# henreedev/audio-pathtracer

Hardware: AMD Instinct MI355X
Metric: rays/sec + IR-frames/sec (1s IR, depth 8) (higher is better)
Workload: dtype f32

## Files before the change

### audio-pathtracer_amd/csrc/fs_aux_kernels.hip

```cpp
#include "fs_dev_trav.hpp"
#include "fs_dev_walk.hpp"
#include "fs_dev_coop.hpp"
#include "fs_dev_recon.hpp"
#include "fs_launch.hpp"

namespace fs {
namespace {

template <bool SPECTRAL>
__global__ __launch_bounds__(kBlock) void reconstruct_kernel(const float* __restrict__ energy, int B, int nb,
                                                             int num_samples, int spb, float* __restrict__ ir_bands,
                                                             float* __restrict__ ir_mono, const float* __restrict__ carrier) {
    extern __shared__ __attribute__((aligned(16))) float s_amp[];
    if (SPECTRAL && (int)blockIdx.y == B) {
        reconstruct_spectral_row((int)blockIdx.x, energy, B, nb, num_samples, spb, ir_bands, ir_mono, s_amp, nullptr, nullptr, carrier);
        return;
    }
    reconstruct_body_fast((int)blockIdx.y, (int)blockIdx.x, energy, B, nb, num_samples, spb, ir_bands, ir_mono, s_amp, nullptr);
}

template <bool SPECTRAL>
__global__ __launch_bounds__(kBlock) void reconstruct_batch_kernel(const ReconItem* __restrict__ table, int B, int nb, int num_samples,
                                                                   uint32_t cb, PublishWord pub, const float* __restrict__ carrier) {
    extern __shared__ __attribute__((aligned(16))) float s_rb[];
// ... 244 lines not shown
                    finished = false;
                }
            }
            if (finished) {
                if (is_occl) { acc->occlusion = de; mode = DONE; }
                else { if (de > 0.0f) { ++direct_hits; direct_sum += de; } mode = MAIN; }
            }
        }
    }
    if (mine && !is_occl) {
        if (result > 0.0f) atomicAdd(&acc->reaching, 1u);
        if (direct_hits) { atomicAdd(&acc->direct_hits, direct_hits); atomicAdd(&acc->direct_energy_sum, direct_sum); }
    }
    if (traces) atomicAdd(&acc->traces, traces);
}

__global__ void add_energy_kernel(float* row, int nb, float delay, float e) {
    float x = (delay * 1000.f) / 1.0f;
    float fl = floorf(x);
    int bin = !(fl > 0.0f) ? 0 : (fl >= (float)(nb - 1) ? nb - 1 : (int)fl);
    row[bin] += e;
}

}

void launch_reconstruct(const float* energy, int B, int num_bins, int sample_rate, int num_samples, int spb,
                        float* ir_bands, float* ir_mono, hipStream_t s, const float* carrier) {
    (void)sample_rate;
    int chunks = (num_samples + kChunk - 1) / kChunk;
    dim3 grid((chunks + kBlock - 1) / kBlock, B + 1);
    const size_t lds = recon_lds_bytes(num_bins);
    if (carrier) {
        allow_lds(reconstruct_kernel<true>, lds);
        hipLaunchKernelGGL(reconstruct_kernel<true>, grid, dim3(kBlock), lds, s, energy, B, num_bins, num_samples, spb, ir_bands, ir_mono, carrier);
    } else {
        allow_lds(reconstruct_kernel<false>, lds);
        hipLaunchKernelGGL(reconstruct_kernel<false>, grid, dim3(kBlock), lds, s, energy, B, num_bins, num_samples, spb, ir_bands, ir_mono, nullptr);
    }
}

void launch_reconstruct_batch(const ReconItem* table, int count, int B, int num_bins, int num_samples, hipStream_t s, const PublishWord& pub,
                              const float* carrier, float* const* room, float bin_duration) {
    if (count <= 0) return;
    const uint32_t chunks = (uint32_t)((num_samples + kChunk - 1) / kChunk), cb = (chunks + kBlock - 1) / kBlock;
    const size_t lds = recon_lds_bytes(num_bins);
    bool spectral = false;
// ... 101 lines not shown
```

### audio-pathtracer_amd/csrc/fs_capi_context.cpp

```cpp
#include "fs_context.hpp"

#include <chrono>

namespace fsi {

Source* get_source(fs_context* ctx, fs_source h) {
    if (h < 0 || (size_t)h >= ctx->sources.size()) return nullptr;
    Source* s = ctx->sources[(size_t)h];
    return (s && s->alive) ? s : nullptr;
}

hipError_t compute_waits_for(fs_context* ctx, hipEvent_t ev) {
    const hipError_t q = hipEventQuery(ev);
    if (q == hipSuccess) { ctx->dbg.waits_skipped++; return hipSuccess; }
    (void)hipGetLastError();
    ctx->dbg.waits_enqueued++;
    return hipStreamWaitEvent(ctx->stream, ev, 0);
}
hipEvent_t tail_batch_event(fs_context* ctx, uint64_t id) {
    const uint64_t newest = ctx->tail_batch_newest.load(std::memory_order_acquire);
    const uint64_t probe = newest - id < (uint64_t)fs_context::kTailBatches ? id : newest - fs_context::kTailBatches + 1;
    return ctx->tail_batch_ev[probe % fs_context::kTailBatches];
}
bool tail_batch_done(fs_context* ctx, uint64_t id) {
// ... 132 lines not shown
    ctx->coop16_nodes = 0; ctx->coop_levels = 0;
    if (ctx->d_tris) (void)hipFree(ctx->d_tris);
    if (ctx->d_tris48) (void)hipFree(ctx->d_tris48);
    if (ctx->d_tri_nrm) (void)hipFree(ctx->d_tri_nrm);
    if (ctx->d_absorption) (void)hipFree(ctx->d_absorption);
    if (ctx->d_leaf_pos) (void)hipFree(ctx->d_leaf_pos);
    if (ctx->d_node_box) (void)hipFree(ctx->d_node_box);
    if (ctx->d_move) (void)hipFree(ctx->d_move);
    ctx->d_leaf_pos = nullptr; ctx->d_node_box = nullptr; ctx->d_move = nullptr;
    ctx->move_cap = 0;
    ctx->refit_pending = false;
    ctx->d_nodes = nullptr; ctx->d_tris = nullptr; ctx->d_absorption = nullptr;
    ctx->d_tris48 = nullptr; ctx->d_tri_nrm = nullptr;
    if (ctx->deep.buf) (void)hipFree(ctx->deep.buf);
    for (int32_t* b : ctx->deep.retired) (void)hipFree(b);
    ctx->deep = DeepStore{};
    ctx->scene = DeviceScene{};
    ctx->committed = false;
}

void free_state(fs_context* ctx) {
    if (ctx->st.end_pos) (void)hipFree(ctx->st.end_pos);
    if (ctx->st.end_misc) (void)hipFree(ctx->st.end_misc);
    if (ctx->st.seg_np) (void)hipFree(ctx->st.seg_np);
    if (ctx->st.seg_mat) (void)hipFree(ctx->st.seg_mat);
    if (ctx->d_seg_pos) (void)hipFree(ctx->d_seg_pos);
    ctx->d_seg_pos = nullptr; ctx->cap_pos = 0;
    if (ctx->st.slot_of) (void)hipFree(ctx->st.slot_of);
    for (void* q : {(void*)ctx->d_over_np, (void*)ctx->d_over_mat, (void*)ctx->d_over_pos, (void*)ctx->d_cont, (void*)ctx->d_end_posd})
        if (q) (void)hipFree(q);
    if (ctx->h_overflow) (void)hipHostFree(ctx->h_overflow);
    ctx->h_overflow = nullptr;
    ctx->d_over_np = nullptr; ctx->d_over_mat = nullptr; ctx->d_over_pos = nullptr; ctx->d_overflow = nullptr; ctx->d_cont = nullptr; ctx->d_end_posd = nullptr;
    ctx->over_cap = ctx->over_cap_pos = 0; ctx->cap_posd = 0;
    if (ctx->walk.perm) (void)hipFree(ctx->walk.perm);
    ctx->walk.perm = nullptr;
    ctx->st = SubpathState{};
    ctx->cap_lanes = ctx->cap_seg = 0;
}

hipEvent_t take_event(fs_context* ctx) {
    if (!ctx->free_events.empty()) {
        hipEvent_t e = ctx->free_events.back();
        ctx->free_events.pop_back();
        return e;
    }
// ... 67 lines not shown
        want_cap = (uint32_t)std::min<size_t>(lanes, std::max<size_t>(ctx->over_cap, (size_t)(4.0 * tail * (double)lanes) + 64));
        if (ctx->over_cap_forced > 0) want_cap = std::max(ctx->over_cap, (uint32_t)ctx->over_cap_forced);
    }
    const bool new_sets = sets != ctx->state_sets || staged != ctx->state_cont;
    const bool grow_lanes = lanes > ctx->cap_lanes || new_sets;
    const bool grow_seg = seg > ctx->cap_seg || grow_lanes;
    const bool grow_over = unbounded && (want_cap > ctx->over_cap || !ctx->d_over_np || new_sets);
    const bool grow_over_pos = unbounded && want_positions && (want_cap > ctx->over_cap_pos || !ctx->d_over_pos);
    const bool grow_pos = want > ctx->cap_pos;
    if (grow_lanes || grow_seg || grow_over || grow_over_pos || grow_pos) {
        FS_FLUSH(ctx);
        FS_HIP(ctx, hipStreamSynchronize(ctx->stream));
    }
    if (grow_pos) {
        if (ctx->d_seg_pos) (void)hipFree(ctx->d_seg_pos);
        ctx->d_seg_pos = nullptr; ctx->cap_pos = 0;
        FS_HIP(ctx, hipMalloc((void**)&ctx->d_seg_pos, sizeof(float4) * std::max<size_t>(want, 1)));
        ctx->cap_pos = want;
    }
    if (grow_lanes) {
        lanes = std::max(lanes, ctx->cap_lanes);
        if (ctx->st.end_pos) (void)hipFree(ctx->st.end_pos);
        if (ctx->st.end_misc) (void)hipFree(ctx->st.end_misc);
        if (ctx->st.slot_of) (void)hipFree(ctx->st.slot_of);
        if (ctx->walk.perm) (void)hipFree(ctx->walk.perm);
        if (ctx->d_cont) (void)hipFree(ctx->d_cont);
        ctx->st.end_pos = nullptr; ctx->st.end_misc = nullptr; ctx->st.slot_of = nullptr; ctx->d_cont = nullptr;
        ctx->walk.perm = nullptr;
        ctx->cap_lanes = 0;
        FS_HIP(ctx, hipMalloc((void**)&ctx->st.end_pos, sizeof(float4) * (size_t)sets * lanes));
        FS_HIP(ctx, hipMalloc((void**)&ctx->st.end_misc, sizeof(uint2) * (size_t)sets * lanes));
        FS_HIP(ctx, hipMalloc((void**)&ctx->st.slot_of, sizeof(uint32_t) * (size_t)sets * lanes));
        if (staged) FS_HIP(ctx, hipMalloc((void**)&ctx->d_cont, sizeof(float4) * 2 * (size_t)sets * lanes));
        ctx->cap_seg = 0;
        ctx->cap_lanes = lanes;
        ctx->state_sets = sets;
        ctx->state_cont = staged;
    }
    if (grow_seg) {
        seg = std::max(seg, (size_t)levels * ctx->cap_lanes);
        if (ctx->st.seg_np) (void)hipFree(ctx->st.seg_np);
        if (ctx->st.seg_mat) (void)hipFree(ctx->st.seg_mat);
        ctx->st.seg_np = nullptr; ctx->st.seg_mat = nullptr;
        ctx->cap_seg = 0;
        FS_HIP(ctx, hipMalloc((void**)&ctx->st.seg_np, sizeof(float2) * (size_t)ctx->state_sets * seg));
        FS_HIP(ctx, hipMalloc((void**)&ctx->st.seg_mat, sizeof(uint32_t) * (size_t)ctx->state_sets * seg));
        if (ctx->walk.perm) (void)hipFree(ctx->walk.perm);
        ctx->walk.perm = nullptr;
        ctx->perm_words = seg + ctx->cap_lanes;
        FS_HIP(ctx, hipMalloc((void**)&ctx->walk.perm, sizeof(uint32_t) * (size_t)ctx->state_sets * ctx->perm_words));
        ctx->cap_seg = seg;
    }
    if (!ctx->d_overflow) {
        FS_HIP(ctx, hipHostMalloc((void**)&ctx->h_overflow, 64, hipHostMallocDefault));
// ... 389 lines not shown
```

### audio-pathtracer_amd/csrc/fs_capi_frame.cpp

```cpp
#include "fs_context.hpp"

namespace {

int ensure_energy_buffer(fs_context* ctx, Source* s, int b) {
    if (s->d_energy[b]) return FS_OK;
    const size_t eb = sizeof(float) * (size_t)ctx->cfg.num_bands * (size_t)ctx->num_bins;
    FS_HIP(ctx, hipMalloc((void**)&s->d_energy[b], eb));
    FS_HIP(ctx, hipMemsetAsync(s->d_energy[b], 0, eb, ctx->stream));
    if (!s->ev_rec[b]) FS_HIP(ctx, hipEventCreateWithFlags(&s->ev_rec[b], kDeviceEventFlags));
    if (!s->ev_red[b]) FS_HIP(ctx, hipEventCreateWithFlags(&s->ev_red[b], kDeviceEventFlags));
    return FS_OK;
}

struct Frame {
    Source* const* srcs = nullptr;
    int count = 0;
    const fs_params* p = nullptr;
    const fs_context::GroupEntry* group = nullptr;
    KParams kp{};
    int B = 1, levels = 0;
    bool batch = false, unbounded = false, all_conn = false, mis = false, fixed = false, accumulate = false, pipe_ok = false;
    bool dir = false;
    DirArgs dargs{};
    std::vector<WalkStage> stages;
// ... 109 lines not shown
        std::vector<int> own_bound;
        const bool lane = (ctx->coop_info.wide16.rec != nullptr || ctx->coop_info.wide4.rec != nullptr) && sync_lane_plan(ctx, kp, &f.lane_len, &lane_bound);
        if (!lane) f.lane_len = 0;
        if (lane && ctx->sync_stage_bounds_default && lane_bound > 0) own_bound.push_back(lane_bound);
        for (int bound : own_bound.empty() ? ctx->sync_stage_bounds : own_bound) { WalkStage sr; sr.begin = begin; sr.end = bound; f.stages.push_back(sr); begin = bound; }
        WalkStage last; last.begin = begin; last.end = 1 << 30;
        f.stages.push_back(last);
    } else {
        f.stages.push_back(WalkStage());
    }
}

int frame_resources(fs_context* ctx, Frame& f) {
    KParams& kp = f.kp;
    const int B = f.B, count = f.count;
    const bool staged = f.stages.size() > 1;
    int rc = ensure_state(ctx, kp.num_local, f.levels, f.unbounded, (double)f.p->rr_prob, f.all_conn, f.mis,
                          (int)f.stages.size() + 2, staged);
    if (rc) return rc;
    f.fidx = ctx->frame_index;
    const size_t set = f.fidx % (unsigned)ctx->state_sets;
    SubpathState& st = f.st;
    st = ctx->st;
    st.end_pos += set * ctx->cap_lanes; st.end_misc += set * ctx->cap_lanes; st.slot_of += set * ctx->cap_lanes;
    st.seg_np += set * ctx->cap_seg; st.seg_mat += set * ctx->cap_seg;
    st.cont_a = staged ? ctx->d_cont + 2 * set * ctx->cap_lanes : nullptr;
    st.cont_b = staged ? st.cont_a + ctx->cap_lanes : nullptr;
    st.end_posd = nullptr;
    if (kp.dpos) {
        const size_t lanes = 2 * (size_t)kp.num_local;
        if (lanes > ctx->cap_posd) {
            FS_HIP(ctx, hipStreamSynchronize(ctx->stream));
            if (ctx->d_end_posd) (void)hipFree(ctx->d_end_posd);
            ctx->d_end_posd = nullptr; ctx->cap_posd = 0;
            FS_HIP(ctx, hipMalloc((void**)&ctx->d_end_posd, sizeof(double) * 3 * lanes));
            ctx->cap_posd = lanes;
        }
        st.end_posd = ctx->d_end_posd;
    }
    f.scratch = ctx->walk.queue_head + (size_t)(f.fidx % kScratchSets) * kScratchAllocWords;
    f.perm_buf = ctx->walk.perm ? ctx->walk.perm + set * ctx->perm_words : nullptr;
    st.seg_pos = f.all_conn ? ctx->d_seg_pos : nullptr;
    st.seg_nrm = f.mis ? ctx->d_seg_pos + (size_t)f.levels * 2 * (size_t)kp.num_local : nullptr;
    st.main_levels = f.levels;
    st.over_levels = f.unbounded ? kOverLevels : 0;
    st.over_cap = f.unbounded ? ctx->over_cap : 0;
    st.over_np = ctx->d_over_np ? ctx->d_over_np + set * (size_t)kOverLevels * ctx->over_cap : nullptr;
// ... 657 lines not shown
```

### audio-pathtracer_amd/csrc/fs_capi_scene.cpp

```cpp
#include "fs_context.hpp"

static int update_triangles(fs_context* ctx, int32_t first, int32_t count, const float* xyz, bool new_rest);

namespace fsi {

void cancel_refine(fs_context* ctx) {
    if (ctx->refine) ctx->refine->cancel.store(true, std::memory_order_relaxed);
    ctx->refine.reset();
    ctx->moved_since_refine = false;
}
void wait_refine(const std::shared_ptr<RefineJob>& j) {
    std::unique_lock<std::mutex> l(j->mu);
    j->cv.wait(l, [&] { return j->done; });
}
void join_refine_threads(fs_context* ctx) {
    for (std::thread& t : ctx->refine_threads)
        if (t.joinable()) t.join();
    ctx->refine_threads.clear();
}

static inline void transform_vertex(const float* a, const float* r, float* w) {
    const float x = r[0], y = r[1], z = r[2];
    for (int k = 0; k < 3; ++k) w[k] = ((a[4 * k] * x + a[4 * k + 1] * y) + a[4 * k + 2] * z) + a[4 * k + 3];
}
// ... 94 lines not shown
}

int fs_scene_set_materials(fs_context* ctx, const float* absorption, const float* transmission,
                           const float* scattering, int32_t M, int32_t B) {
    if (!ctx) return FS_ERR_INVALID_ARGUMENT;
    if (M < 0 || (M > 0 && !absorption) || M >= (int32_t)FS_NO_MATERIAL)
        return ctx->fail(FS_ERR_INVALID_ARGUMENT, "bad material table");
    if (B != ctx->cfg.num_bands) return ctx->fail(FS_ERR_SIZE_MISMATCH, "material bands != context num_bands");
    size_t n = (size_t)M * (size_t)B;
    ctx->h_absorption.assign(absorption, absorption + n);
    if (transmission) ctx->h_transmission.assign(transmission, transmission + n); else ctx->h_transmission.clear();
    if (scattering) ctx->h_scattering.assign(scattering, scattering + n); else ctx->h_scattering.clear();
    ctx->M = M;
    ctx->committed = false;
    return FS_OK;
}

static int upload_materials(fs_context* ctx) {
    const size_t mb = ctx->h_absorption.size() * sizeof(float);
    if (mb) {
        const int B = ctx->cfg.num_bands, M = ctx->M;
        std::vector<float> table(ctx->h_absorption);
        table.resize((size_t)M * B + (size_t)M * 3 * B + (size_t)M * 3, 0.f);
        float* gain = table.data() + (size_t)M * B;
        float* prob = gain + (size_t)M * 3 * B;
        const bool has_t = ctx->h_transmission.size() == (size_t)M * B, has_s = ctx->h_scattering.size() == (size_t)M * B;
        for (int m = 0; m < M; ++m) {
            float sum[3] = {0.f, 0.f, 0.f};
            for (int b = 0; b < B; ++b) {
                const float alpha = ctx->h_absorption[(size_t)m * B + b];
                float tau = has_t ? ctx->h_transmission[(size_t)m * B + b] : 0.0f;
                const float sigma = has_s ? ctx->h_scattering[(size_t)m * B + b] : 1.0f;
                const float refl = 1.0f - alpha;
                if (refl + tau > 1.0f) tau = 1.0f - refl;
                float g[3] = {refl * sigma, refl * (1.0f - sigma), tau};
                for (int l = 0; l < 3; ++l) {
                    if (!(g[l] > 0.0f)) g[l] = 0.0f;
                    gain[((size_t)m * 3 + l) * B + b] = g[l];
                    sum[l] += g[l];
                }
            }
            float mean[3], tot = 0.0f;
            for (int l = 0; l < 3; ++l) { mean[l] = sum[l] / (float)B; tot += mean[l]; }
            for (int l = 0; l < 3; ++l) prob[(size_t)m * 3 + l] = tot > 0.0f ? mean[l] / tot : (l == 0 ? 1.0f : 0.0f);
        }
        FS_HIP(ctx, hipMalloc((void**)&ctx->d_absorption, table.size() * sizeof(float)));
        FS_HIP(ctx, hipMemcpy(ctx->d_absorption, table.data(), table.size() * sizeof(float), hipMemcpyHostToDevice));
    }
    return FS_OK;
}

static int pack_scene(fs_context* ctx, size_t count, size_t cap) {
    if (!ctx->d_tris48) {
        FS_HIP(ctx, hipMalloc((void**)&ctx->d_tris48, std::max<size_t>(cap, 1) * sizeof(Tri48)));
        FS_HIP(ctx, hipMalloc((void**)&ctx->d_tri_nrm, std::max<size_t>(cap, 1) * sizeof(float4)));
    }
    launch_pack_triangles(ctx->d_tris, (int)count, ctx->d_tris48, ctx->d_tri_nrm, ctx->stream);
    FS_HIP(ctx, hipGetLastError());
    return FS_OK;
}

static int refresh_coop_nodes(fs_context* ctx, bool topology_changed) {
    const size_t n = ctx->bvh.nodes.size();
    const int levels = (int)ctx->bvh.level_begin.size() - 1;
    ctx->coop_info = CoopInfo{};
    ctx->scene.coop_info = &ctx->coop_info;
    if (n == 0 || levels < 1 || levels > kMaxBuildLevels) return FS_OK;
    if (n > ctx->coop_cap) {
        if (ctx->d_coop) { FS_HIP(ctx, hipStreamSynchronize(ctx->stream)); (void)hipFree(ctx->d_coop); }
        ctx->d_coop = nullptr; ctx->coop_cap = 0;
// ... 22 lines not shown
    }
    launch_coop_nodes(ctx->d_nodes, (int)n, ctx->d_coop, ctx->stream);
    launch_coop16(ctx->d_coop, ctx->d_coop_levels, ctx->d_coop_levels + (kMaxBuildLevels + 2), ctx->coop_levels, ctx->coop16_nodes, ctx->d_coop16, ctx->stream);
    FS_HIP(ctx, hipGetLastError());
    ctx->coop_info.wide16 = CoopView{ctx->d_coop16, 0, ctx->coop16_nodes, 4, (int16_t)(15 * ((ctx->coop_levels + 1) / 2) + 1)};
    ctx->coop_info.wide4 = CoopView{ctx->d_coop, 0, (int32_t)n, 2, (int16_t)(std::max(ctx->bvh.stack_need, 2) + 4)};
    if (ctx->amax > kCoopMaxCoordinate) { ctx->coop_info.wide16.rec = nullptr; ctx->coop_info.wide4.rec = nullptr; }
    static const bool dbg_info = std::getenv("FS_DEBUG_SCENE_INFO") != nullptr;
    if (dbg_info)
        std::fprintf(stderr, "[frequensee] tree: %zu 4-wide nodes in %d levels -> %d 16-wide nodes\n", n, levels, ctx->coop16_nodes);
    return FS_OK;
}

static int finish_commit(fs_context* ctx, size_t scene_bytes) {
    object_moves_after_commit(ctx);
    ctx->amax = 0.f;
    for (float v : ctx->h_xyz) ctx->amax = std::max(ctx->amax, std::fabs(v));
    ctx->scene.nodes = ctx->d_nodes;
    ctx->scene.tris = ctx->d_tris48;
    ctx->scene.tri_nrm = ctx->d_tri_nrm;
    ctx->scene.absorption = ctx->d_absorption;
    ctx->scene.lobe_gain = ctx->d_absorption ? ctx->d_absorption + (size_t)ctx->M * ctx->cfg.num_bands : nullptr;
    ctx->scene.lobe_prob = ctx->d_absorption ? ctx->scene.lobe_gain + (size_t)ctx->M * 3 * ctx->cfg.num_bands : nullptr;
    ctx->scene.num_nodes = (int32_t)ctx->bvh.nodes.size();
    ctx->scene.num_tris = ctx->T;
    ctx->scene.num_materials = ctx->M;
    const int worst = std::max(ctx->bvh.stack_need, 2) + kStackSlack;
    int deep_rows = 0;
    if (worst <= ctx->stack_rows_cap + 1) {
        ctx->scene.stack_rows = worst; ctx->scene.stack_limit = worst; ctx->scene.stack_attn = 0x7FFFFFFFu;
    } else {
        ctx->scene.stack_rows = ctx->stack_rows_cap + 1; ctx->scene.stack_limit = ctx->stack_rows_cap;
        ctx->scene.stack_attn = (uint32_t)(ctx->stack_rows_cap - 4);
        deep_rows = ((worst + kDeepChunk - 1) / kDeepChunk) * kDeepChunk + kDeepChunk;
    }
    if (deep_rows != ctx->deep.rows) {
        if (ctx->deep.buf) (void)hipFree(ctx->deep.buf);
        for (int32_t* b : ctx->deep.retired) (void)hipFree(b);
        ctx->deep = DeepStore{};
        ctx->deep.rows = deep_rows;
    }
    ctx->scene.stack_worst = traversal_lds_bytes(worst, ctx->cfg.num_bands, ctx->num_bins) <= ctx->lds_limit ? worst : 0;
    ctx->scene.deep = nullptr; ctx->scene.deep_lanes = 0;
    ctx->scene.deep_owner = &ctx->deep;
    ctx->stats.bvh_nodes = (uint32_t)ctx->bvh.nodes.size();
    ctx->stats.triangles = (uint32_t)ctx->T;
// ... 407 lines not shown
    FS_HIP(ctx, fold_moved_amax(ctx));
    const size_t nodes = ctx->bvh.nodes.size(), T = (size_t)ctx->T;
    const size_t levels = ctx->bvh.level_begin.empty() ? 0 : ctx->bvh.level_begin.size() - 1;
    uint32_t hdr[12] = {(uint32_t)nodes, (uint32_t)T, (uint32_t)levels, (uint32_t)ctx->bvh.stack_need, 0, 0,
                        (uint32_t)ctx->coop16_nodes, (uint32_t)ctx->coop_levels, ctx->refit_pending ? 1u : 0u,
                        ctx->fast_cap_tris > 0 ? 1u : 0u, 0, 0};
    std::memcpy(&hdr[4], &ctx->bvh.pad, sizeof(float));
    std::memcpy(&hdr[5], &ctx->amax, sizeof(float));
    const void* src = nullptr;
    bool on_device = true;
    size_t need = 0;
    switch (what) {
        case 0: src = hdr; need = sizeof(hdr); on_device = false; break;
        case 1: src = ctx->d_nodes; need = nodes * sizeof(NodeQ4); break;
        case 2: src = ctx->d_tris; need = T * sizeof(Tri64); break;
        case 3: src = ctx->d_tris48; need = T * sizeof(Tri48); break;
        case 4: src = ctx->d_tri_nrm; need = T * sizeof(float4); break;
        case 5: src = ctx->d_leaf_pos; need = T * sizeof(uint32_t); break;
        case 6: src = ctx->bvh.level_begin.data(); need = ctx->bvh.level_begin.size() * sizeof(int32_t); on_device = false; break;
        case 7: src = ctx->d_coop; need = 4 * nodes * sizeof(CoopChild); break;
        case 8: src = ctx->d_coop16; need = 16 * (size_t)ctx->coop16_nodes * sizeof(CoopChild); break;
        case 9: src = ctx->d_coop_levels; need = ctx->d_coop_levels ? 2 * (size_t)(kMaxBuildLevels + 2) * sizeof(int32_t) : 0; break;
        case 10: src = ctx->d_node_box; need = 2 * nodes * sizeof(float4); break;
        default: return ctx->fail(FS_ERR_INVALID_ARGUMENT, "fs_debug_scene_snapshot: no such array");
    }
    *bytes = need;
    if (need == 0) return FS_OK;
    if (!src) return ctx->fail(FS_ERR_INVALID_ARGUMENT, "fs_debug_scene_snapshot: the scene holds no such array");
    if (!out || cap < need) return ctx->fail(FS_ERR_SIZE_MISMATCH, "fs_debug_scene_snapshot: buffer too small");
    if (on_device) FS_HIP(ctx, hipMemcpy(out, src, need, hipMemcpyDeviceToHost));
    else std::memcpy(out, src, need);
    return FS_OK;
}

int fs_scene_set_objects(fs_context* ctx, const uint32_t* object_id, int32_t T) {
    if (!ctx) return FS_ERR_INVALID_ARGUMENT;
    if (object_id && T != ctx->T) return ctx->fail(FS_ERR_SIZE_MISMATCH, "object ids: T != number of triangles");
    if (object_id) ctx->h_obj.assign(object_id, object_id + T);
    else ctx->h_obj.clear();
    ctx->committed = false;
    return FS_OK;
}

}
```

### audio-pathtracer_amd/csrc/fs_dev_common.hpp

```cpp
#pragma once
#include <algorithm>
#include <atomic>

#include "fs_internal.hpp"

namespace fs {
namespace {

constexpr float kPi = 3.1415926535897932f;
constexpr uint32_t kNoMat = FS_NO_MATERIAL;
constexpr uint32_t kLobeDiffuse = 0u, kLobeSpecular = 1u, kLobeTransmit = 2u;
constexpr int kLobeShift = 16;
constexpr int kDone = (int)0x80000000;
constexpr uint32_t kMissKey = 0xFFFFFFFCu;
constexpr double kFixedScale = 1099511627776.0;
#ifdef FS_WAVE_TIMELINE
__device__ unsigned long long* g_wave_buf;
__device__ unsigned long long* g_conn_buf;
#endif
#ifdef FS_TRAV_STATS
__device__ unsigned long long g_trav_stats[32];
__device__ unsigned short* g_step_buf;
#endif

// ... 129 lines not shown
    const bool inside = (det != 0.0f) & (us >= 0.0f) & (us <= ad) & (vs >= 0.0f) & ((us + vs) <= ad);
    if (!inside) return false;
    float t = tn / det;
    t_out = t;
    return (t > 0.0f) & (t <= tmax);
}


template <int B> struct Bands { static constexpr int kMax = B ? B : FS_MAX_BANDS; };
template <int B> __device__ __forceinline__ int band_count(const KParams& kp) { return B ? B : kp.num_bands; }

template <int B, int LOBES = -1>
__device__ __forceinline__ void apply_segment(float (&E)[Bands<B>::kMax], float nd, uint32_t mat, float prob, const KParams& kp,
                                              const DeviceScene& sc) {
    const int NB = band_count<B>(kp);
    const bool lobes = LOBES < 0 ? kp.lobes != 0 : LOBES != 0;
    if (nd < kp.min_seg) return;
    float nd2 = nd * nd;
    float geo = 1.0f / (4 * kPi * nd2);
    float pw = powf(prob, kp.prob_exponent);
    const uint32_t lobe = (lobes && mat != kNoMat) ? ((mat >> kLobeShift) & 3u) : 0u;
    if (lobes && mat != kNoMat) mat &= 0xFFFFu;
    bool has = (mat != kNoMat) && ((int32_t)mat < sc.num_materials);
    const float* coeff = lobes ? sc.lobe_gain + ((size_t)mat * 3 + lobe) * NB : sc.absorption + (size_t)mat * NB;
    const bool over_pi = !lobes || lobe == kLobeDiffuse;
#pragma unroll
    for (int b = 0; b < Bands<B>::kMax; ++b) {
        if (B == 0 && b >= NB) break;
        float bsdf = 1.0f;
        if (has) bsdf = over_pi ? coeff[b] / kPi : coeff[b];
        float e = E[b];
        e *= bsdf;
        e *= geo;
        e *= expf(-kp.air[b] * nd);
        e /= pw;
        E[b] = e;
    }
}

template <int B>
struct SegFactors { float geo, pw; bool live; float bsdf[Bands<B>::kMax], ex[Bands<B>::kMax]; };
template <int B, int LOBES = -1>
__device__ __forceinline__ void segment_factors(SegFactors<B>& f, float nd, uint32_t mat, float prob, const KParams& kp, const DeviceScene& sc) {
    const int NB = band_count<B>(kp);
    const bool lobes = LOBES < 0 ? kp.lobes != 0 : LOBES != 0;
    f.live = !(nd < kp.min_seg);
    float nd2 = nd * nd;
    f.geo = 1.0f / (4 * kPi * nd2);
    f.pw = powf(prob, kp.prob_exponent);
    const uint32_t lobe = (lobes && mat != kNoMat) ? ((mat >> kLobeShift) & 3u) : 0u;
    if (lobes && mat != kNoMat) mat &= 0xFFFFu;
    bool has = (mat != kNoMat) && ((int32_t)mat < sc.num_materials);
    const float* coeff = lobes ? sc.lobe_gain + ((size_t)mat * 3 + lobe) * NB : sc.absorption + (size_t)mat * NB;
    const bool over_pi = !lobes || lobe == kLobeDiffuse;
#pragma unroll
    for (int b = 0; b < Bands<B>::kMax; ++b) {
        f.bsdf[b] = 1.0f; f.ex[b] = 1.0f;
        if (B == 0 && b >= NB) continue;
        if (has) f.bsdf[b] = over_pi ? coeff[b] / kPi : coeff[b];
        f.ex[b] = expf(-kp.air[b] * nd);
    }
}

}
}
```

### audio-pathtracer_amd/csrc/fs_dev_connect.hpp

```cpp
#pragma once
#include "fs_dev_walk.hpp"

namespace fs {
namespace {

__device__ __forceinline__ int emission_step(const SubpathState& st, uint32_t total, uint32_t sf, int records) {
    for (int j = 0; j < records; ++j)
        if (load_np(st, total, j, sf).x != 0.0f) return j;
    return -1;
}
__device__ __forceinline__ void emission_ray(const KParams& kp, uint32_t li, int step, float& wx, float& wy, float& wz) {
    const uint32_t sid = li / kp.pairs_per_source;
    const uint32_t pair = kp.pair_begin + (li - sid * kp.pairs_per_source);
    const uint32_t seed = kp.item_seeds > 0 ? item_seed_lo(kp, sid) : kp.seed_lo;
    const uint32_t bs = (uint32_t)step << 1;
    const uint4 r = philox(pair, bs, 0, seed, kp.seed_hi);
    sample_sphere(pair, bs, r, seed, kp.seed_hi, wx, wy, wz);
}
struct DirLookup { const float* row; int K, k; float t; };
__device__ __forceinline__ DirLookup dir_lookup(const Directivity& d, float wx, float wy, float wz) {
    DirLookup L;
    L.row = d.table; L.K = d.samples; L.k = 0; L.t = 0.0f;
    if (!d.table) return L;
    const float fx = d.fwd[0], fy = d.fwd[1], fz = d.fwd[2];
// ... 28 lines not shown
#ifdef FS_WAVE_TIMELINE
    unsigned long long tl[6] = {__builtin_amdgcn_s_memrealtime(), 0, 0, 0, 0, 0};
#endif
    for (int i = threadIdx.x; i < NB * W; i += kBlock) s_hist[i] = 0.0f;
    if (threadIdx.x == 0) { s_lo = nb; s_hi = -1; s_dep = 0u; s_tst = 0u; s_sgs = 0u; }
    if (bid == 0u)
        for (int i = threadIdx.x; i < 1 + 2 * kPlanBuckets; i += kBlock) queue_head[i] = 0u;
    __syncthreads();

    const uint32_t n = kp.num_local;
    const uint32_t total = 2u * n;
    unsigned my_deposits = 0, my_tested = 0, my_segments = 0;
    uint32_t cnt_nv = 0u, cnt_nt = 0u;
    const uint32_t ppw = (uint32_t)pairs_per_wave, per_block = ppw * (kBlock / 64);
    const uint32_t lane = threadIdx.x & 63u, wave = threadIdx.x >> 6;

    auto chunk = [&](uint32_t first, uint32_t end, unsigned long long* fixed_dst, float* far_dst) {
        const uint32_t li = first + wave * ppw + lane;
        const bool active = lane < ppw && li < end;
        const uint32_t lc = active ? li : 0u;
        const uint32_t sf = slot_of(st, lc), sl = slot_of(st, n + lc);
        const float4 F = st.end_pos[sf];
        const uint2 Fm = st.end_misc[sf];
        const float4 L = st.end_pos[sl];
        const uint2 Lm = st.end_misc[sl];
        float dx = L.x - F.x, dy = L.y - F.y, dz = L.z - F.z;
        float l2 = dx * dx + dy * dy + dz * dz;
        float len = sqrtf(l2);
        float inv = 1.0f / len;
        float tmax = len - kp.connect_pullback;
        float ux = dx * inv, uy = dy * inv, uz = dz * inv;
        float conn_nd = 0.0f;
        if (EXT && kp.dpos) {
            const double* Fd = st.end_posd + 3 * (size_t)sf;
            const double* Ld = st.end_posd + 3 * (size_t)sl;
            const double ex = Ld[0] - Fd[0], ey = Ld[1] - Fd[1], ez = Ld[2] - Fd[2];
            const double e2 = ex * ex + ey * ey + ez * ez;
            const double elen = sqrt(e2), einv = 1.0 / elen;
            l2 = e2 > 1e-8f ? 1.0f : 0.0f;
            ux = (float)(ex * einv); uy = (float)(ey * einv); uz = (float)(ez * einv);
            tmax = (float)(elen - kp.connect_pullback);
            conn_nd = (float)(elen / (double)kp.dist_divisor);
        }
        bool has_ray = active && (l2 > 1e-8f) && (tmax > 0.0f);
        Ray ray = make_ray(F.x, F.y, F.z, ux, uy, uz);
        bool sphere_blocked = false;
        if (EXT && has_ray && (kp.listener_radius > 0.0f || kp.source_radius > 0.0f)) {
            float ts;
            if (kp.listener_radius > 0.0f && sphere_hit(ray, kp.lis, kp.listener_radius, tmax, ts)) sphere_blocked = true;
            if (kp.source_radius > 0.0f) {
                float c[3] = {kp.src[0], kp.src[1], kp.src[2]};
                if (kp.src_table) { const uint32_t sid = lc / kp.pairs_per_source; c[0] = kp.src_table[4 * sid]; c[1] = kp.src_table[4 * sid + 1]; c[2] = kp.src_table[4 * sid + 2]; }
                if (sphere_hit(ray, c, kp.source_radius, tmax, ts)) sphere_blocked = true;
            }
            if (sphere_blocked) has_ray = false;
        }
#ifdef FS_WAVE_TIMELINE
        if (!tl[1]) tl[1] = __builtin_amdgcn_s_memrealtime();
#endif
        my_tested += active ? 1u : 0u;
        my_segments += active ? Fm.y + Lm.y : 0u;
        const bool hit = trav_any_shared<COUNT>(sc, has_ray, ray, tmax, &s_stack[threadIdx.x], s_share, &cnt_nv, &cnt_nt);
#ifdef FS_WAVE_TIMELINE
        if (!tl[2]) tl[2] = __builtin_amdgcn_s_memrealtime();
#endif
        float E[Bands<B>::kMax];
#pragma unroll
        for (int b = 0; b < Bands<B>::kMax; ++b) E[b] = 1.0f;
        float sd = 0.0f;
        auto eval_alone = [&]() {
        const int kf = (int)Fm.y, kl = (int)Lm.y;
        if (AHEAD > 1) {
            for (int j0 = 0; j0 < kf; j0 += AHEAD) {
                float2 np[AHEAD];
                uint32_t mt[AHEAD];
#pragma unroll
                for (int u = 0; u < AHEAD; ++u) { const int j = min(j0 + u, kf - 1); np[u] = load_np(st, total, j, sf); mt[u] = load_mat(st, total, j, sf); }
#pragma unroll
                for (int u = 0; u < AHEAD; ++u)
                    if (j0 + u < kf) { sd += np[u].x; apply_segment<B, LOBES>(E, np[u].x, mt[u], np[u].y, kp, sc); }
            }
        } else
        for (int j = 0; j < kf; ++j) {
            const float2 np = load_np(st, total, j, sf);
            sd += np.x;
// ... 202 lines not shown
```

### audio-pathtracer_amd/csrc/fs_dev_walk.hpp

```cpp
#pragma once
#include "fs_dev_trav.hpp"

namespace fs {
namespace {

struct Walker {
    uint32_t g, slot, side, li, pair;
    int k;
    float px, py, pz, nx, ny, nz;
    double dpx, dpy, dpz;
    bool has_normal;
    bool arrived;
    uint32_t mat;
    uint32_t lobe;
    float prob, prob_new;
    uint32_t ign;
};

__device__ __forceinline__ uint32_t item_seed_lo(const KParams& kp, uint32_t sid) {
    uint32_t s = kp.seed_lo;
    if (kp.item_seeds > 0) {
        s = kp.item_seed[0];
        s = sid == 1u ? kp.item_seed[1] : s;
        s = sid == 2u ? kp.item_seed[2] : s;
// ... 14 lines not shown
    return rec_in_main(st, k) ? st.seg_np[rec_main(total, k, slot)] : st.over_np[rec_over(st, k, slot)];
}
__device__ __forceinline__ uint32_t load_mat(const SubpathState& st, uint32_t total, int k, uint32_t slot) {
    return rec_in_main(st, k) ? st.seg_mat[rec_main(total, k, slot)] : st.over_mat[rec_over(st, k, slot)];
}
__device__ __forceinline__ float4 load_pos(const SubpathState& st, uint32_t total, int k, uint32_t slot) {
    return rec_in_main(st, k) ? st.seg_pos[rec_main(total, k, slot)] : st.over_pos[rec_over(st, k, slot)];
}
__device__ __forceinline__ float4 load_nrm(const SubpathState& st, uint32_t total, int k, uint32_t slot) {
    return rec_in_main(st, k) ? st.seg_nrm[rec_main(total, k, slot)] : st.over_nrm[rec_over(st, k, slot)];
}
__device__ __forceinline__ void store_mat(const SubpathState& st, uint32_t total, int k, uint32_t slot, uint32_t v) {
    if (rec_in_main(st, k)) st.seg_mat[rec_main(total, k, slot)] = v;
    else if (rec_fits(st, k, slot)) st.over_mat[rec_over(st, k, slot)] = v;
}
__device__ __forceinline__ uint32_t slot_of(const SubpathState& st, uint32_t g) { return st.slot_of ? st.slot_of[g] : g; }

__device__ __forceinline__ void walker_start(Walker& w, uint32_t g, uint32_t slot, const KParams& kp, const SubpathState& st,
                                             bool own = true) {
    const uint32_t n = kp.num_local;
    w.g = g;
    w.slot = slot;
    if (own && st.slot_of) st.slot_of[g] = slot;
    w.side = g >= n ? 1u : 0u;
    w.li = g - w.side * n;
    w.pair = kp.pair_begin + w.li;
    w.px = w.side ? kp.lis[0] : kp.src[0];
    w.py = w.side ? kp.lis[1] : kp.src[1];
    w.pz = w.side ? kp.lis[2] : kp.src[2];
    if (kp.src_table) {
        const uint32_t sid = w.li / kp.pairs_per_source;
        w.pair = kp.pair_begin + (w.li - sid * kp.pairs_per_source);
        if (!w.side) { w.px = kp.src_table[4 * sid]; w.py = kp.src_table[4 * sid + 1]; w.pz = kp.src_table[4 * sid + 2]; }
    }
    w.ign = w.side ? kp.lis_object : kp.src_object;
    if (kp.src_table && !w.side) w.ign = __float_as_uint(kp.src_table[4 * (w.li / kp.pairs_per_source) + 3]);
    w.dpx = (double)w.px; w.dpy = (double)w.py; w.dpz = (double)w.pz;
    w.nx = 0.f; w.ny = 0.f; w.nz = 0.f;
    w.has_normal = false;
    w.arrived = false;
    w.lobe = 0u;
    w.mat = kNoMat;
    w.prob = 1.0f; w.prob_new = 1.0f;
    w.k = 0;
}

// ... 64 lines not shown
    if (!(t > 0.0f)) t = sq - b;
    if (!(t > 0.0f && t <= tmax)) return false;
    t_out = t;
    return true;
}
__device__ __forceinline__ void sphere_normal(const Ray& r, float t, const float c[3], float& nx, float& ny, float& nz) {
    float x = fmaf(t, r.dx, r.ox) - c[0], y = fmaf(t, r.dy, r.oy) - c[1], z = fmaf(t, r.dz, r.oz) - c[2];
    float l2 = x * x + y * y + z * z;
    float inv = 1.0f / sqrtf(l2);
    x = x * inv; y = y * inv; z = z * inv;
    float dn = fmaf(x, r.dx, fmaf(y, r.dy, z * r.dz));
    if (dn > 0.0f) { x = -x; y = -y; z = -z; }
    nx = x; ny = y; nz = z;
}

template <bool EXT = false>
__device__ __forceinline__ void walker_apply_hit(Walker& w, const KParams& kp, const DeviceScene& sc,
                                                 const SubpathState& st, const Ray& ray, const Trav& T, const float4* surf = nullptr) {
    float qx = w.px, qy = w.py, qz = w.pz;
    double dqx = w.dpx, dqy = w.dpy, dqz = w.dpz;
    uint32_t mat_new = w.mat;
    bool hit = T.leaf_index >= 0;
    float t = T.t;
    if (hit && surf) {
        float x = surf->x, y = surf->y, z = surf->z;
        const float dn = fmaf(x, ray.dx, fmaf(y, ray.dy, z * ray.dz));
        if (dn > 0.0f) { x = -x; y = -y; z = -z; }
        w.nx = x; w.ny = y; w.nz = z;
        mat_new = __float_as_uint(surf->w);
    } else if (hit) hit_surface(sc, T.leaf_index, ray, w.nx, w.ny, w.nz, mat_new);
    const float other_radius = !EXT ? 0.0f : (w.side ? kp.source_radius : kp.listener_radius);
    if (EXT && other_radius > 0.0f) {
        float c[3] = {w.side ? kp.src[0] : kp.lis[0], w.side ? kp.src[1] : kp.lis[1], w.side ? kp.src[2] : kp.lis[2]};
        if (w.side && kp.src_table) {
            const uint32_t sid = w.li / kp.pairs_per_source;
            c[0] = kp.src_table[4 * sid]; c[1] = kp.src_table[4 * sid + 1]; c[2] = kp.src_table[4 * sid + 2];
        }
        float ts;
        if (sphere_hit(ray, c, other_radius, kp.max_trace_dist, ts) && (!hit || ts <= t)) {
            hit = true; t = ts;
            sphere_normal(ray, ts, c, w.nx, w.ny, w.nz);
            mat_new = kNoMat;
        }
    }
    const bool DPOS = EXT && kp.dpos != 0;
    if (hit) {
        if (DPOS) {
            const bool shifted = ray.ox != w.px || ray.oy != w.py || ray.oz != w.pz;
            const double ipx = (shifted ? (double)ray.ox : w.dpx) + (double)t * (double)ray.dx;
            const double ipy = (shifted ? (double)ray.oy : w.dpy) + (double)t * (double)ray.dy;
            const double ipz = (shifted ? (double)ray.oz : w.dpz) + (double)t * (double)ray.dz;
            dqx = ipx + (double)kp.surface_offset * (double)w.nx;
            dqy = ipy + (double)kp.surface_offset * (double)w.ny;
            dqz = ipz + (double)kp.surface_offset * (double)w.nz;
            qx = (float)dqx; qy = (float)dqy; qz = (float)dqz;
        } else {
            qx = fmaf(kp.surface_offset, w.nx, fmaf(t, ray.dx, ray.ox));
            qy = fmaf(kp.surface_offset, w.ny, fmaf(t, ray.dy, ray.oy));
            qz = fmaf(kp.surface_offset, w.nz, fmaf(t, ray.dz, ray.oz));
        }
        w.has_normal = true;
    }
    w.arrived = hit;
    float nd;
    if (DPOS) {
        const double ex = dqx - w.dpx, ey = dqy - w.dpy, ez = dqz - w.dpz;
        nd = (float)(sqrt(ex * ex + ey * ey + ez * ez) / (double)kp.dist_divisor);
    } else {
        float ddx = qx - w.px, ddy = qy - w.py, ddz = qz - w.pz;
        float dist = sqrtf(ddx * ddx + ddy * ddy + ddz * ddz);
        nd = dist / kp.dist_divisor;
    }
    const float2 rec_np = w.side == 0 ? make_float2(nd, w.prob) : make_float2(nd, w.prob_new);
    const uint32_t rec_mat = w.side == 0 ? (w.mat | w.lobe) : mat_new;
    if (rec_in_main(st, w.k)) {
        const size_t r = rec_main(2u * kp.num_local, w.k, w.slot);
        st.seg_np[r] = rec_np;
        st.seg_mat[r] = rec_mat;
        if (st.seg_pos) st.seg_pos[r] = make_float4(qx, qy, qz, 0.0f);
        if (st.seg_nrm) st.seg_nrm[r] = make_float4(w.nx, w.ny, w.nz, 0.0f);
    } else if (rec_fits(st, w.k, w.slot)) {
        const size_t r = rec_over(st, w.k, w.slot);
        st.over_np[r] = rec_np;
        st.over_mat[r] = rec_mat;
// ... 304 lines not shown
```

### audio-pathtracer_amd/csrc/fs_internal.hpp

```cpp
#pragma once

#include <hip/hip_runtime.h>

#include <atomic>
#include <cstdint>
#include <string>
#include <vector>

#include "../../include/frequensee.h"

#if defined(FS_TRAV_STATS) && !defined(FS_EXPERIMENTS)
#define FS_EXPERIMENTS
#endif

namespace fs {

struct alignas(16) NodeQ4 {
    float ox, oy, oz;
    float sx;
    uint32_t lox, loy, loz, hix;
    uint32_t hiy, hiz;
    float sy, sz;
    int32_t child[4];
};
// ... 28 lines not shown
constexpr int kBlock = 256;
constexpr int kChunk = 16;
constexpr int kReconBlockSamples = kBlock * kChunk;
constexpr int kWarm = 96;
constexpr size_t recon_lds_bytes(int num_bins, bool fast = true) {
    return sizeof(float) * ((size_t)num_bins + (fast ? (size_t)kReconBlockSamples + kWarm : 0) + (size_t)kBlock * (kChunk + 1));
}
constexpr size_t kReconStaticLdsReserve = 4096;
constexpr int max_recon_bins(size_t lds) {
    return lds > recon_lds_bytes(0) + kReconStaticLdsReserve ? (int)((lds - recon_lds_bytes(0) - kReconStaticLdsReserve) / sizeof(float)) : 0;
}
static_assert(64 % kChunk == 0, "carrier_stride (below) must hold whole chunks");
constexpr int kHistWindow = 256;
constexpr int kUnboundedDepth = 1 << 24;
constexpr int kOverLevels = 448;

struct DeviceScene {
    const NodeQ4* nodes;
    const Tri48* tris;
    const float4* tri_nrm;
    const float* absorption;
    const float* lobe_gain;
    const float* lobe_prob;
    int32_t num_nodes;
    int32_t num_tris;
    int32_t num_materials;
    int32_t stack_rows;
    int32_t stack_limit;
    uint32_t stack_attn;
    int32_t stack_worst;
    const struct CoopInfo* coop_info;
    int32_t* deep;
    uint32_t deep_lanes;
    struct DeepStore* deep_owner;
};

struct KParams {
    uint32_t seed_lo, seed_hi;
    uint32_t pair_begin;
    uint32_t num_local;
    uint32_t pairs_per_source;
    const float* src_table;
    uint32_t src_object, lis_object;
    uint32_t item_seed[4];
    int32_t item_seeds;
    int32_t depth;
// ... 25 lines not shown
    int32_t samples;
    const float* table;
};
struct DirArgs {
    Directivity one;
    const Directivity* tab;
};

struct SoundKParams {
    uint32_t seed_lo, seed_hi;
    int32_t raycasts_per_tick, raycast_bounces;
    float raycast_distance, simulated_duration, listener_radius;
    float src[3], lis[3];
};
struct SoundAccum {
    unsigned long long traces;
    unsigned reaching, direct_hits;
    float direct_energy_sum, occlusion;
};

struct SubpathState {
    float4* end_pos;
    uint2* end_misc;
    float2* seg_np;
    uint32_t* seg_mat;
    float4* seg_pos;
    float4* seg_nrm;
    uint32_t* slot_of;
    float2* over_np; uint32_t* over_mat; float4* over_pos; float4* over_nrm;
    unsigned* overflow;
    uint32_t over_cap;
    int32_t main_levels, over_levels;
    float4* cont_a; float4* cont_b;
    double* end_posd;
};
constexpr uint32_t kContHasNormal = 1u << 16, kContArrived = 1u << 17, kContAlive = 1u << 18;

struct WalkStage {
    int32_t begin = 0, end = 1 << 30;
    uint32_t slots_cap = 0xFFFFFFFFu;
};
struct WalkLane {
    int32_t len = 0;
    uint32_t cap = 0;
    int32_t begin = 0, end = 1 << 30;
    int32_t mode = 0;
// ... 270 lines not shown
    const float* in;
    float* out;
    float* mix;
};
void launch_reflect_render(const ReflectRenderBatch& b, hipStream_t s);
void launch_add_energy(float* energy_row, int num_bins, float delay_s, float e, hipStream_t s);
size_t traversal_lds_bytes(int stack_rows, int bands, int num_bins);
int default_hist_window(int bands);
constexpr int kOneShotMaxRanks = 16;
constexpr size_t kOneShotHeaderBytes = 256;
struct OneShotView {
    void* mail[kOneShotMaxRanks];
    int32_t world, rank;
    size_t slot_bytes;
};
void launch_oneshot_reduce(const OneShotView& v, void* buffer, int words, bool u64, int set, uint32_t seq, unsigned* err,
                           hipStream_t s);
void launch_update_triangles(Tri64* tris, Tri48* packed, float4* nrm, const uint32_t* leaf_pos, int first, int count,
                             const float* xyz, hipStream_t s);
void launch_transform_objects(Tri64* tris, Tri48* packed, float4* nrm, const uint32_t* leaf_pos, const float* rest,
                              const uint32_t* csr, const uint32_t* prefix, const uint32_t* start, const float* m, int n,
                              uint32_t total, uint32_t* amax_bits, hipStream_t s);
void launch_pack_triangles(const Tri64* tris, int count, Tri48* packed, float4* nrm, hipStream_t s);
void launch_refit(NodeQ4* nodes, const Tri64* tris, float4* node_box, const int32_t* level_begin, int levels, float pad,
                  hipStream_t s);
void launch_coop_nodes(const NodeQ4* nodes, int n, CoopChild* out, hipStream_t s);
void launch_coop16(const CoopChild* in, const int32_t* level_begin_dev, const int32_t* dense_dev, int levels, int n16, CoopChild* out, hipStream_t s);
constexpr int kMaxBuildLevels = 96;
struct DeviceBuildInfo {
    int32_t num_nodes, levels, stack_need, reserved;
    int32_t level_begin[kMaxBuildLevels + 1];
};
size_t device_build_scratch_bytes(int T);
bool launch_device_build(const float* xyz, const uint16_t* mat, const uint32_t* object_id, int T, const float lo[3],
                         const float hi[3], NodeQ4* nodes, Tri64* tris, uint32_t* leaf_pos, void* scratch, size_t scratch_bytes,
                         DeviceBuildInfo* info_dev, hipStream_t s);
constexpr int kFftChunkLog = 11;
void launch_apply_material_fd(const float* in, int L, int n, float2* x, float2* y, const float2* W, const float* resp,
                              float* out, hipStream_t s);
constexpr uint64_t kCarrierSeed = 0x5EED;
constexpr int kCarrierMaxLog = 24;
struct CarrierBands { int32_t lo[FS_MAX_BANDS + 1]; };
__host__ __device__ constexpr int carrier_stride(int num_samples) { return (num_samples + 63) / 64 * 64; }
void launch_build_carriers(int B, int n, int N, int ld, const CarrierBands& bands, float2* X, float2* y, const float2* W,
                           const float* zeros, float* out, hipStream_t s);

// ... 2 lines not shown
```

Before: 988.8 million.

## Precompute material BSDF divided by pi and pre-test endpoint own triangles in connect

Adds a device kernel at scene upload that stores absorption/pi and diffuse lobe gain/pi tables, so per-bounce BSDF evaluation reads a precomputed quotient instead of dividing by pi. Separately, walk kernels now record the triangle each subpath endpoint sits on, and the connect kernel tests the connection ray against both endpoint triangles before BVH traversal, marking the ray blocked early if either hits. The triangle bookkeeping costs an extra per-lane array, extra global stores in the walk, and two triangle tests per connection. It may also change results if the self-hit test disagrees with what the old traversal reported.

```diff
diff --git a/audio-pathtracer_amd/csrc/fs_aux_kernels.hip b/audio-pathtracer_amd/csrc/fs_aux_kernels.hip
--- a/audio-pathtracer_amd/csrc/fs_aux_kernels.hip
+++ b/audio-pathtracer_amd/csrc/fs_aux_kernels.hip
@@ -290,6 +290,20 @@
     row[bin] += e;
 }
 
+__global__ void material_quotients_kernel(const float* __restrict__ absorption, const float* __restrict__ lobe_gain, int M, int B,
+                                          float* __restrict__ out) {
+    const int i = (int)(blockIdx.x * blockDim.x + threadIdx.x);
+    if (i >= M * B) return;
+    const int m = i / B, b = i - m * B;
+    out[i] = absorption[i] / kPi;
+    out[(size_t)M * B + i] = lobe_gain[((size_t)m * 3 + kLobeDiffuse) * B + b] / kPi;
+}
+
+}
+
+void launch_material_quotients(const float* absorption, const float* lobe_gain, int M, int B, float* out, hipStream_t s) {
+    if (M * B <= 0) return;
+    hipLaunchKernelGGL(material_quotients_kernel, dim3((unsigned)((M * B + kBlock - 1) / kBlock)), dim3(kBlock), 0, s, absorption, lobe_gain, M, B, out);
 }
 
 void launch_reconstruct(const float* energy, int B, int num_bins, int sample_rate, int num_samples, int spb,
diff --git a/audio-pathtracer_amd/csrc/fs_capi_context.cpp b/audio-pathtracer_amd/csrc/fs_capi_context.cpp
--- a/audio-pathtracer_amd/csrc/fs_capi_context.cpp
+++ b/audio-pathtracer_amd/csrc/fs_capi_context.cpp
@@ -178,6 +178,7 @@
 void free_state(fs_context* ctx) {
     if (ctx->st.end_pos) (void)hipFree(ctx->st.end_pos);
     if (ctx->st.end_misc) (void)hipFree(ctx->st.end_misc);
+    if (ctx->st.end_tri) (void)hipFree(ctx->st.end_tri);
     if (ctx->st.seg_np) (void)hipFree(ctx->st.seg_np);
     if (ctx->st.seg_mat) (void)hipFree(ctx->st.seg_mat);
     if (ctx->d_seg_pos) (void)hipFree(ctx->d_seg_pos);
@@ -291,14 +292,16 @@
         lanes = std::max(lanes, ctx->cap_lanes);
         if (ctx->st.end_pos) (void)hipFree(ctx->st.end_pos);
         if (ctx->st.end_misc) (void)hipFree(ctx->st.end_misc);
+        if (ctx->st.end_tri) (void)hipFree(ctx->st.end_tri);
         if (ctx->st.slot_of) (void)hipFree(ctx->st.slot_of);
         if (ctx->walk.perm) (void)hipFree(ctx->walk.perm);
         if (ctx->d_cont) (void)hipFree(ctx->d_cont);
-        ctx->st.end_pos = nullptr; ctx->st.end_misc = nullptr; ctx->st.slot_of = nullptr; ctx->d_cont = nullptr;
+        ctx->st.end_pos = nullptr; ctx->st.end_misc = nullptr; ctx->st.end_tri = nullptr; ctx->st.slot_of = nullptr; ctx->d_cont = nullptr;
         ctx->walk.perm = nullptr;
         ctx->cap_lanes = 0;
         FS_HIP(ctx, hipMalloc((void**)&ctx->st.end_pos, sizeof(float4) * (size_t)sets * lanes));
         FS_HIP(ctx, hipMalloc((void**)&ctx->st.end_misc, sizeof(uint2) * (size_t)sets * lanes));
+        FS_HIP(ctx, hipMalloc((void**)&ctx->st.end_tri, sizeof(int32_t) * (size_t)sets * lanes));
         FS_HIP(ctx, hipMalloc((void**)&ctx->st.slot_of, sizeof(uint32_t) * (size_t)sets * lanes));
         if (staged) FS_HIP(ctx, hipMalloc((void**)&ctx->d_cont, sizeof(float4) * 2 * (size_t)sets * lanes));
         ctx->cap_seg = 0;
diff --git a/audio-pathtracer_amd/csrc/fs_capi_frame.cpp b/audio-pathtracer_amd/csrc/fs_capi_frame.cpp
--- a/audio-pathtracer_amd/csrc/fs_capi_frame.cpp
+++ b/audio-pathtracer_amd/csrc/fs_capi_frame.cpp
@@ -155,7 +155,7 @@
     const size_t set = f.fidx % (unsigned)ctx->state_sets;
     SubpathState& st = f.st;
     st = ctx->st;
-    st.end_pos += set * ctx->cap_lanes; st.end_misc += set * ctx->cap_lanes; st.slot_of += set * ctx->cap_lanes;
+    st.end_pos += set * ctx->cap_lanes; st.end_misc += set * ctx->cap_lanes; st.end_tri += set * ctx->cap_lanes; st.slot_of += set * ctx->cap_lanes;
     st.seg_np += set * ctx->cap_seg; st.seg_mat += set * ctx->cap_seg;
     st.cont_a = staged ? ctx->d_cont + 2 * set * ctx->cap_lanes : nullptr;
     st.cont_b = staged ? st.cont_a + ctx->cap_lanes : nullptr;
diff --git a/audio-pathtracer_amd/csrc/fs_capi_scene.cpp b/audio-pathtracer_amd/csrc/fs_capi_scene.cpp
--- a/audio-pathtracer_amd/csrc/fs_capi_scene.cpp
+++ b/audio-pathtracer_amd/csrc/fs_capi_scene.cpp
@@ -140,6 +140,7 @@
         const int B = ctx->cfg.num_bands, M = ctx->M;
         std::vector<float> table(ctx->h_absorption);
         table.resize((size_t)M * B + (size_t)M * 3 * B + (size_t)M * 3, 0.f);
+        const size_t quot = table.size();
         float* gain = table.data() + (size_t)M * B;
         float* prob = gain + (size_t)M * 3 * B;
         const bool has_t = ctx->h_transmission.size() == (size_t)M * B, has_s = ctx->h_scattering.size() == (size_t)M * B;
@@ -162,8 +163,10 @@
             for (int l = 0; l < 3; ++l) { mean[l] = sum[l] / (float)B; tot += mean[l]; }
             for (int l = 0; l < 3; ++l) prob[(size_t)m * 3 + l] = tot > 0.0f ? mean[l] / tot : (l == 0 ? 1.0f : 0.0f);
         }
-        FS_HIP(ctx, hipMalloc((void**)&ctx->d_absorption, table.size() * sizeof(float)));
-        FS_HIP(ctx, hipMemcpy(ctx->d_absorption, table.data(), table.size() * sizeof(float), hipMemcpyHostToDevice));
+        FS_HIP(ctx, hipMalloc((void**)&ctx->d_absorption, (quot + 2 * (size_t)M * B) * sizeof(float)));
+        FS_HIP(ctx, hipMemcpy(ctx->d_absorption, table.data(), quot * sizeof(float), hipMemcpyHostToDevice));
+        launch_material_quotients(ctx->d_absorption, ctx->d_absorption + (size_t)M * B, M, B, ctx->d_absorption + quot, ctx->stream);
+        FS_HIP(ctx, hipGetLastError());
     }
     return FS_OK;
 }
@@ -232,6 +235,7 @@
     ctx->scene.absorption = ctx->d_absorption;
     ctx->scene.lobe_gain = ctx->d_absorption ? ctx->d_absorption + (size_t)ctx->M * ctx->cfg.num_bands : nullptr;
     ctx->scene.lobe_prob = ctx->d_absorption ? ctx->scene.lobe_gain + (size_t)ctx->M * 3 * ctx->cfg.num_bands : nullptr;
+    ctx->scene.over_pi = ctx->d_absorption ? ctx->scene.lobe_prob + (size_t)ctx->M * 3 : nullptr;
     ctx->scene.num_nodes = (int32_t)ctx->bvh.nodes.size();
     ctx->scene.num_tris = ctx->T;
     ctx->scene.num_materials = ctx->M;
@@ -685,6 +689,7 @@
         case 8: src = ctx->d_coop16; need = 16 * (size_t)ctx->coop16_nodes * sizeof(CoopChild); break;
         case 9: src = ctx->d_coop_levels; need = ctx->d_coop_levels ? 2 * (size_t)(kMaxBuildLevels + 2) * sizeof(int32_t) : 0; break;
         case 10: src = ctx->d_node_box; need = 2 * nodes * sizeof(float4); break;
+        case 11: src = ctx->d_absorption; need = ctx->d_absorption ? (6 * (size_t)ctx->M * (size_t)ctx->cfg.num_bands + 3 * (size_t)ctx->M) * sizeof(float) : 0; break;
         default: return ctx->fail(FS_ERR_INVALID_ARGUMENT, "fs_debug_scene_snapshot: no such array");
     }
     *bytes = need;
diff --git a/audio-pathtracer_amd/csrc/fs_dev_common.hpp b/audio-pathtracer_amd/csrc/fs_dev_common.hpp
--- a/audio-pathtracer_amd/csrc/fs_dev_common.hpp
+++ b/audio-pathtracer_amd/csrc/fs_dev_common.hpp
@@ -175,13 +175,13 @@
     const uint32_t lobe = (lobes && mat != kNoMat) ? ((mat >> kLobeShift) & 3u) : 0u;
     if (lobes && mat != kNoMat) mat &= 0xFFFFu;
     bool has = (mat != kNoMat) && ((int32_t)mat < sc.num_materials);
-    const float* coeff = lobes ? sc.lobe_gain + ((size_t)mat * 3 + lobe) * NB : sc.absorption + (size_t)mat * NB;
-    const bool over_pi = !lobes || lobe == kLobeDiffuse;
+    const float* coeff = !lobes ? sc.over_pi + (size_t)mat * NB
+                                : (lobe == kLobeDiffuse ? sc.over_pi + ((size_t)sc.num_materials + mat) * NB : sc.lobe_gain + ((size_t)mat * 3 + lobe) * NB);
 #pragma unroll
     for (int b = 0; b < Bands<B>::kMax; ++b) {
         if (B == 0 && b >= NB) break;
         float bsdf = 1.0f;
-        if (has) bsdf = over_pi ? coeff[b] / kPi : coeff[b];
+        if (has) bsdf = coeff[b];
         float e = E[b];
         e *= bsdf;
         e *= geo;
@@ -204,13 +204,13 @@
     const uint32_t lobe = (lobes && mat != kNoMat) ? ((mat >> kLobeShift) & 3u) : 0u;
     if (lobes && mat != kNoMat) mat &= 0xFFFFu;
     bool has = (mat != kNoMat) && ((int32_t)mat < sc.num_materials);
-    const float* coeff = lobes ? sc.lobe_gain + ((size_t)mat * 3 + lobe) * NB : sc.absorption + (size_t)mat * NB;
-    const bool over_pi = !lobes || lobe == kLobeDiffuse;
+    const float* coeff = !lobes ? sc.over_pi + (size_t)mat * NB
+                                : (lobe == kLobeDiffuse ? sc.over_pi + ((size_t)sc.num_materials + mat) * NB : sc.lobe_gain + ((size_t)mat * 3 + lobe) * NB);
 #pragma unroll
     for (int b = 0; b < Bands<B>::kMax; ++b) {
         f.bsdf[b] = 1.0f; f.ex[b] = 1.0f;
         if (B == 0 && b >= NB) continue;
-        if (has) f.bsdf[b] = over_pi ? coeff[b] / kPi : coeff[b];
+        if (has) f.bsdf[b] = coeff[b];
         f.ex[b] = expf(-kp.air[b] * nd);
     }
 }
diff --git a/audio-pathtracer_amd/csrc/fs_dev_connect.hpp b/audio-pathtracer_amd/csrc/fs_dev_connect.hpp
--- a/audio-pathtracer_amd/csrc/fs_dev_connect.hpp
+++ b/audio-pathtracer_amd/csrc/fs_dev_connect.hpp
@@ -74,8 +74,10 @@
         const uint32_t sf = slot_of(st, lc), sl = slot_of(st, n + lc);
         const float4 F = st.end_pos[sf];
         const uint2 Fm = st.end_misc[sf];
+        const int32_t Ft = st.end_tri[sf];
         const float4 L = st.end_pos[sl];
         const uint2 Lm = st.end_misc[sl];
+        const int32_t Lt = st.end_tri[sl];
         float dx = L.x - F.x, dy = L.y - F.y, dz = L.z - F.z;
         float l2 = dx * dx + dy * dy + dz * dz;
         float len = sqrtf(l2);
@@ -107,12 +109,26 @@
             }
             if (sphere_blocked) has_ray = false;
         }
+        bool own_blocked = false;
+        if (sc.num_tris > 0) {
+            const bool vl = has_ray && (uint32_t)Lt < (uint32_t)sc.num_tris, vf = has_ray && (uint32_t)Ft < (uint32_t)sc.num_tris;
+            const Tri48* tl_ = sc.tris + (vl ? Lt : 0);
+            const Tri48* tf_ = sc.tris + (vf ? Ft : 0);
+            const float4 la = tl_->a, lb = tl_->b, fa = tf_->a, fb = tf_->b;
+            const float lcx = tl_->c.x, fcx = tf_->c.x;
+            float t_l = 0.f, t_f = 0.f;
+            const bool hl = tri_hit(la, lb, make_float4(lcx, 0.f, 0.f, 0.f), ray, tmax, t_l);
+            const bool hf = tri_hit(fa, fb, make_float4(fcx, 0.f, 0.f, 0.f), ray, tmax, t_f);
+            own_blocked = (vl & hl) | (vf & hf);
+            if (COUNT) cnt_nt += (vl ? 1u : 0u) + (vf ? 1u : 0u);
+            if (own_blocked) has_ray = false;
+        }
 #ifdef FS_WAVE_TIMELINE
         if (!tl[1]) tl[1] = __builtin_amdgcn_s_memrealtime();
 #endif
         my_tested += active ? 1u : 0u;
         my_segments += active ? Fm.y + Lm.y : 0u;
-        const bool hit = trav_any_shared<COUNT>(sc, has_ray, ray, tmax, &s_stack[threadIdx.x], s_share, &cnt_nv, &cnt_nt);
+        const bool hit = trav_any_shared<COUNT>(sc, has_ray, ray, tmax, &s_stack[threadIdx.x], s_share, &cnt_nv, &cnt_nt) || own_blocked;
 #ifdef FS_WAVE_TIMELINE
         if (!tl[2]) tl[2] = __builtin_amdgcn_s_memrealtime();
 #endif
diff --git a/audio-pathtracer_amd/csrc/fs_dev_walk.hpp b/audio-pathtracer_amd/csrc/fs_dev_walk.hpp
--- a/audio-pathtracer_amd/csrc/fs_dev_walk.hpp
+++ b/audio-pathtracer_amd/csrc/fs_dev_walk.hpp
@@ -60,6 +60,7 @@
     w.g = g;
     w.slot = slot;
     if (own && st.slot_of) st.slot_of[g] = slot;
+    if (own) st.end_tri[slot] = -1;
     w.side = g >= n ? 1u : 0u;
     w.li = g - w.side * n;
     w.pair = kp.pair_begin + w.li;
@@ -170,6 +171,7 @@
     uint32_t mat_new = w.mat;
     bool hit = T.leaf_index >= 0;
     float t = T.t;
+    int32_t on_tri = T.leaf_index;
     if (hit && surf) {
         float x = surf->x, y = surf->y, z = surf->z;
         const float dn = fmaf(x, ray.dx, fmaf(y, ray.dy, z * ray.dz));
@@ -189,6 +191,7 @@
             hit = true; t = ts;
             sphere_normal(ray, ts, c, w.nx, w.ny, w.nz);
             mat_new = kNoMat;
+            on_tri = -1;
         }
     }
     const bool DPOS = EXT && kp.dpos != 0;
@@ -208,6 +211,7 @@
             qz = fmaf(kp.surface_offset, w.nz, fmaf(t, ray.dz, ray.oz));
         }
         w.has_normal = true;
+        st.end_tri[w.slot] = on_tri;
     }
     w.arrived = hit;
     float nd;
diff --git a/audio-pathtracer_amd/csrc/fs_internal.hpp b/audio-pathtracer_amd/csrc/fs_internal.hpp
--- a/audio-pathtracer_amd/csrc/fs_internal.hpp
+++ b/audio-pathtracer_amd/csrc/fs_internal.hpp
@@ -74,6 +74,7 @@
     const float* absorption;
     const float* lobe_gain;
     const float* lobe_prob;
+    const float* over_pi;
     int32_t num_nodes;
     int32_t num_tris;
     int32_t num_materials;
@@ -145,6 +146,7 @@
 struct SubpathState {
     float4* end_pos;
     uint2* end_misc;
+    int32_t* end_tri;
     float2* seg_np;
     uint32_t* seg_mat;
     float4* seg_pos;
@@ -461,6 +463,7 @@
                               const uint32_t* csr, const uint32_t* prefix, const uint32_t* start, const float* m, int n,
                               uint32_t total, uint32_t* amax_bits, hipStream_t s);
 void launch_pack_triangles(const Tri64* tris, int count, Tri48* packed, float4* nrm, hipStream_t s);
+void launch_material_quotients(const float* absorption, const float* lobe_gain, int M, int B, float* out, hipStream_t s);
 void launch_refit(NodeQ4* nodes, const Tri64* tris, float4* node_box, const int32_t* level_begin, int levels, float pad,
                   hipStream_t s);
 void launch_coop_nodes(const NodeQ4* nodes, int n, CoopChild* out, hipStream_t s);
```

Result: no change. 996.7 million (median of 6 runs) (+0.8%).
